# ezorita/seeq

Measured on AMD Instinct MI355X. Metric: lines/s scanned (20 bp pattern, d=3, 150 bp reads; GB/s in gb_per_s), higher is better.
Workload: dtype int (u16 automaton state ids; exact-pass columns u32 bit-vectors)

## Files before the change

### seeq_amd/csrc/seeq_pair.h

```cpp
#ifndef SEEQ_PAIR_H_
#define SEEQ_PAIR_H_

#define PAIR_X2(K) \
   asm("v_xor_b32_sdwa %0, %1, %2 dst_sel:DWORD dst_unused:UNUSED_PAD src0_sel:DWORD src1_sel:BYTE_" #K : "=v"(ada) : "v"(sa), "v"(ta)); \
   asm("v_xor_b32_sdwa %0, %1, %2 dst_sel:DWORD dst_unused:UNUSED_PAD src0_sel:DWORD src1_sel:BYTE_" #K : "=v"(adb) : "v"(sb), "v"(tb)); \
   sa = *(stream_lds_cu16 *)(uintptr_t)ada; sb = *(stream_lds_cu16 *)(uintptr_t)adb; \
   __builtin_amdgcn_sched_barrier(0);

__device__ __forceinline__ uint32_t pair_prep(uint32_t w)
{
   const uint32_t u = w & 0x06060606u;
   return u | (u << 10);
}

__device__ __forceinline__ void pair_chk(uint32_t w, uint32_t &bad, uint32_t &nm, bool first_of_two)
{
   const uint32_t idx = (w >> 1) & 0x07070707u;
   bad = __builtin_amdgcn_sad_u8(w, __builtin_amdgcn_perm(0x4EFF0AFFu, 0x47544341u, idx), bad);
   const uint32_t nf = __builtin_amdgcn_perm(0x00000100u, 0u, idx);
   nm = first_of_two ? __builtin_amdgcn_udot4(nf, 0x10204080u, nm << 8, false) : __builtin_amdgcn_udot4(nf, 0x01020408u, nm, false);
}

__device__ __forceinline__ void pair_warm4x2(uint32_t &sa, uint32_t wa, uint32_t &sb, uint32_t wb, uint32_t &seena, uint32_t &seenb)
{
   const uint32_t ta = pair_prep(wa), tb = pair_prep(wb);
   uint32_t ada, adb;
   PAIR_X2(1) asm("v_or_b32 %0, %0, %1" : "+v"(seena) : "v"(sa)); asm("v_or_b32 %0, %0, %1" : "+v"(seenb) : "v"(sb));
   PAIR_X2(3) asm("v_or_b32 %0, %0, %1" : "+v"(seena) : "v"(sa)); asm("v_or_b32 %0, %0, %1" : "+v"(seenb) : "v"(sb));
}

template <bool CHK>
__device__ __forceinline__ void pair_own4x2(uint32_t &sa, uint32_t wa, uint32_t &hma, uint32_t &nma, uint32_t &sb, uint32_t wb, uint32_t &hmb, uint32_t &nmb,
                                            uint32_t &bad, bool first_of_two)
{
   const uint32_t ta = pair_prep(wa), tb = pair_prep(wb);
   uint32_t ada, adb;
   PAIR_X2(1)
   asm volatile("" : "+v"(wa));
   if (CHK) pair_chk(wa, bad, nma, first_of_two);
   asm volatile("" : "+v"(bad), "+v"(nma));
   __builtin_amdgcn_sched_barrier(0);
   hma = __builtin_amdgcn_alignbit(sa, hma, 1); hmb = __builtin_amdgcn_alignbit(sb, hmb, 1);
   asm volatile("" : "+v"(hma), "+v"(hmb));
   PAIR_X2(3)
   asm volatile("" : "+v"(wb));
   if (CHK) pair_chk(wb, bad, nmb, first_of_two);
   asm volatile("" : "+v"(bad), "+v"(nmb));
   __builtin_amdgcn_sched_barrier(0);
   hma = __builtin_amdgcn_alignbit(sa, hma, 1); hmb = __builtin_amdgcn_alignbit(sb, hmb, 1);
   asm volatile("" : "+v"(hma), "+v"(hmb));
}

__device__ __forceinline__ uint32_t pair_word8(const fused_v4u &p, const fused_v4u &q, int k)
{
   return k == 0 ? p.x : k == 1 ? p.y : k == 2 ? p.z : k == 3 ? p.w : k == 4 ? q.x : k == 5 ? q.y : k == 6 ? q.z : q.w;
}

typedef uint32_t pair_u32_unaligned __attribute__((aligned(1)));

__device__ __forceinline__ uint32_t pair_nonbase_mask32(const fused_v4u &a, const fused_v4u &b)
{
   const uint32_t w[8] = {a.x, a.y, a.z, a.w, b.x, b.y, b.z, b.w};
   uint32_t h[2];
#pragma unroll
   for (int g = 0; g < 2; g++) {
      uint32_t acc = 0;
#pragma unroll
      for (int k = 4 * g; k < 4 * g + 4; k += 2) {
         uint32_t f[2];
#pragma unroll
         for (int u = 0; u < 2; u++) {
            const uint32_t x = w[k + u];
            const uint32_t t = x ^ __builtin_amdgcn_perm(0x474E5554u, 0x43FF41FFu, x & 0x07070707u);
            f[u] = (((t & 0x5F5F5F5Fu) + 0x7F7F7F7Fu) | t) & 0x80808080u;
         }
         acc = __builtin_amdgcn_udot4(f[0], 0x10204080u, __builtin_amdgcn_udot4(f[1], 0x01020408u, acc << 8, false), false);
      }
      h[g] = acc;
   }
   return (h[0] << 9) | (h[1] >> 7);
}

__device__ __forceinline__ uint32_t pair_count_before(const uint32_t (&m)[4], const uint32_t (&c)[5], uint32_t b)
{
   const uint32_t r = b >> 5, lz = b & 31u;
   const uint32_t mr = r == 0 ? m[0] : r == 1 ? m[1] : r == 2 ? m[2] : r == 3 ? m[3] : 0u;
   const uint32_t cr = r == 0 ? c[0] : r == 1 ? c[1] : r == 2 ? c[2] : r == 3 ? c[3] : c[4];
   return cr + (lz ? (uint32_t)__popc(mr >> (32u - lz)) : 0u);
}

template <int WU, bool CHK>
__device__ __forceinline__ void pair_walk(const fused_v4u (&v)[8], uint32_t halo, bool halo_nl, uint32_t (&hm)[2], uint32_t (&nmask)[4], uint32_t &tile_bad)
{
   constexpr int NQ = 8, NM = 4;
   uint32_t sa = 0, sb = 0, hma = 0, hmb = 0, seena = 0, seenb = 0, bad = 0, nma = 0, nmb = 0;
#pragma unroll
   for (int k = 8 - WU; k < 8; k++)
      pair_warm4x2(sa, stream_from_prev_lane(pair_word8(v[NQ - 2], v[NQ - 1], k), halo_nl ? 0x0A0A0A0Au : (uint32_t)__builtin_amdgcn_readlane((int)halo, k)),
                        sb, pair_word8(v[NQ / 2 - 2], v[NQ / 2 - 1], k), seena, seenb);
#pragma unroll
   for (int q = 0; q < NQ / 2; q++) {
      pair_own4x2<CHK>(sa, v[q].x, hma, nma, sb, v[q + NQ / 2].x, hmb, nmb, bad, true);
      pair_own4x2<CHK>(sa, v[q].y, hma, nma, sb, v[q + NQ / 2].y, hmb, nmb, bad, false);
      pair_own4x2<CHK>(sa, v[q].z, hma, nma, sb, v[q + NQ / 2].z, hmb, nmb, bad, true);
      pair_own4x2<CHK>(sa, v[q].w, hma, nma, sb, v[q + NQ / 2].w, hmb, nmb, bad, false);
      if (CHK && (q & 1)) { nmask[q >> 1] = nma; nmask[(q >> 1) + NM / 2] = nmb; nma = 0; nmb = 0; }
   }
   tile_bad = bad;
   hm[0] = __builtin_bitreverse32(hma) | ((seena & 1u) << 31);
   hm[1] = __builtin_bitreverse32(hmb) | ((seenb & 1u) << 31);
}

template <int WU, bool FA, bool IG = false, bool LL = false>
__global__ __launch_bounds__(64 * STREAM_NW, 8) void k_pair(FusedArgs a)
{
   static_assert(!(FA && IG), "SQ_IGNORE on FASTA input stays with k_stream");
   static_assert(!(LL && (FA || IG)), "the long-line variant serves plain text under SQ_FAIL / SQ_CONVERT");
   constexpr int NW = STREAM_NW;
   constexpr int CH = 128;
   constexpr int NQ = CH / 16;
   constexpr int NM = CH / 32;
   constexpr uint32_t TB = 64u * CH;
   static_assert(WU >= 4 && WU <= 8, "warm-up is 16 .. 32 bytes");
   extern __shared__ __align__(16) uint8_t dsmem[];
   const int tid = threadIdx.x, lane = tid & 63;
   const int wave = __builtin_amdgcn_readfirstlane(tid >> 6);
   {
      const fused_v4u *src = reinterpret_cast<const fused_v4u *>(a.dfa);
      for (uint32_t i = tid; i < a.dfa_rows; i += 64 * NW) reinterpret_cast<fused_v4u *>(dsmem)[i] = src[i];
   }
   __syncthreads();

   const uint32_t gwave = blockIdx.x * NW + wave, nwaves = gridDim.x * NW;
   if (a.clk_probe != nullptr && blockIdx.x == 0 && tid == 0) { a.clk_probe[0] = __builtin_readcyclecounter(); a.clk_probe[1] = wall_clock64(); }
   uint32_t wv_lines = 0, wv_hitlines = 0, wv_hdrs = 0, slice_pos = 0;
   bool wv_overflow = false;
   uint32_t wv_dirty = 0, wv_lastnl = 0;
   uint32_t dmode = 0;
   uint4 *slice = a.tmp + (size_t)gwave * a.slice_cap;
   const uint64_t lim = a.seg_base + a.seg_len;
   const uint64_t last = a.nbytes - 1;

   fused_v4u v[NQ];
   uint32_t halo = 0;
   uint32_t tile = gwave;
   while (tile < a.ntiles) {
      const uint64_t t0 = a.seg_base + (uint64_t)tile * TB;
      const bool partial = tile + 1 == a.ntiles && (a.seg_len % TB) != 0;
      const uint32_t next = tile + nwaves;
      uint32_t lane_off = (uint32_t)lane * CH;
      asm volatile("" : "+v"(lane_off));
      const uint64_t my = t0 + lane_off;
      {
         if (!partial) {
            const uint8_t *p = a.text + my;
#pragma unroll
            for (int q = 0; q < NQ; q++) v[q] = *reinterpret_cast<const fused_v4u_unaligned *>(p + 16 * q);
            uint32_t lid;
            asm volatile("v_mbcnt_lo_u32_b32 %0, -1, 0\n\tv_mbcnt_hi_u32_b32 %0, -1, %0" : "=v"(lid));
            halo = *reinterpret_cast<const pair_u32_unaligned *>(a.text + (t0 >= 32 ? t0 - 32 : 0) + ((lid & 7u) << 2));
         } else {
#pragma unroll
            for (int q = 0; q < NQ; q++) v[q] = dfa_load16(a.text, my + 16 * q, lim);
            const fused_v4u h0 = dfa_load16(a.text, t0 >= 32 ? t0 - 32 : 0, lim), h1 = dfa_load16(a.text, t0 >= 32 ? t0 - 16 : 0, lim);
            halo = pair_word8(h0, h1, 0);
#pragma unroll
            for (int k = 1; k < 8; k++) halo = (lane & 7) == k ? pair_word8(h0, h1, k) : halo;
         }
      }
      const bool halo_nl = t0 < 32;
      uint32_t hm[2], nmask[NM];
      if (!dmode) {
         uint32_t tile_bad;
         pair_walk<WU, true>(v, halo, halo_nl, hm, nmask, tile_bad);
         const uint64_t badlanes = __ballot(tile_bad != 0);
         dmode = (uint32_t)__builtin_amdgcn_readfirstlane(badlanes != 0 ? 1 : 0);
         if (LL && lane == 0) { a.tile_dirty[tile] = badlanes != 0 ? 1u : 0u; a.tile_dmask[tile] = badlanes; }
      } else {
         uint32_t unused;
         pair_walk<WU, false>(v, halo, halo_nl, hm, nmask, unused);
         if (LL && lane == 0) { a.tile_dirty[tile] = 1u; a.tile_dmask[tile] = ~0ull; }
      }
      if (dmode) {
         wv_dirty |= 1u;
#pragma unroll
         for (int r = 0; r < NM; r++) nmask[r] = stream_nl_mask32(v[2 * r], v[2 * r + 1], false);
      }
      uint32_t valid = CH;
      if (partial) {
         valid = lim > my ? (lim - my < CH ? (uint32_t)(lim - my) : (uint32_t)CH) : 0u;
#pragma unroll
         for (int r = 0; r < NM; r++) {
            const uint32_t lo = 32u * r;
            nmask[r] &= valid <= lo ? 0u : (valid >= lo + 32 ? 0xFFFFFFFFu : ~(0xFFFFFFFFu >> (valid - lo)));
         }
#pragma unroll
         for (int x = 0; x < 2; x++) {
            const uint32_t vx = valid <= 64u * x ? 0u : (valid - 64u * x >= 64u ? 64u : valid - 64u * x);
            const uint32_t np = (vx + 1u) >> 1;
            hm[x] &= np >= 32u ? 0xFFFFFFFFu : ~(0xFFFFFFFFu >> np);
         }
      }
      uint32_t mk[2] = {0u, 0u};
      const uint32_t walk_hm[2] = {hm[0], hm[1]};
      if (IG) {
         uint32_t e_tail = 0;
         if (t0 <= last && last < t0 + TB) { if (a.text[last] != '\n') e_tail = (uint32_t)(last - t0) + 1u; }
         else if (!partial && a.text[t0 + TB] == '\n') e_tail = TB;
         e_tail = (uint32_t)__builtin_amdgcn_readfirstlane((int)e_tail);
         uint32_t vm[NM], sk[NM], dn[NM];
#pragma unroll
         for (int r = 0; r < NM; r++) {
            const uint32_t lo = 32u * r;
            vm[r] = valid <= lo ? 0u : (valid >= lo + 32 ? 0xFFFFFFFFu : ~(0xFFFFFFFFu >> (valid - lo)));
            sk[r] = dmode ? pair_nonbase_mask32(v[2 * r], v[2 * r + 1]) & ~nmask[r] & vm[r] : 0u;
            dn[r] = ~(nmask[r] | sk[r]) & vm[r];
         }
         uint32_t cD[5], cS[5];
         cD[0] = 0; cS[0] = 0;
#pragma unroll
         for (int r = 0; r < NM; r++) { cD[r + 1] = cD[r] + (uint32_t)__popc(dn[r]); cS[r + 1] = cS[r] + (uint32_t)__popc(sk[r]); }
         const uint32_t end_after = (uint32_t)__builtin_amdgcn_update_dpp(0, (int)(nmask[0] >> 31), 0x130, 0xf, 0xf, true);
         uint32_t b_tail = 0;
         if (e_tail && (uint32_t)lane == (e_tail - 1u) / CH) b_tail = e_tail - (uint32_t)lane * CH;
         if (end_after) b_tail = CH;
         uint32_t baseD = 0, baseS = 0, seen_end = 0, firstP = 0, first_pq = 0;
         auto mark = [&](uint32_t pq) { if (pq < 32u) mk[0] |= 0x80000000u >> pq; else mk[1] |= 0x80000000u >> (pq - 32u); };
         auto line_end = [&](uint32_t b, uint32_t Dc, uint32_t Sc) {
            if (b >= 1u) {
               const uint32_t lineD = Dc + baseD, lineS = Sc + baseS;
               if (!seen_end) { firstP = 0x80000000u | (lineS << 14) | lineD; first_pq = (b - 1u) >> 1; }
               else if (lineS != 0u && lineD >= a.ig_thr) mark((b - 1u) >> 1);
            }
            baseD = 0u - Dc; baseS = 0u - Sc; seen_end = 1u;
         };
#pragma unroll
         for (int r = 0; r < NM; r++) {
            uint32_t mm = nmask[r];
            while (mm) {
               const uint32_t lz = (uint32_t)__builtin_clz(mm);
               mm &= ~(0x80000000u >> lz);
               line_end(32u * r + lz, cD[r] + (uint32_t)__popc((dn[r] >> 1) >> (31u - lz)), cS[r] + (uint32_t)__popc((sk[r] >> 1) >> (31u - lz)));
            }
         }
         if (__ballot(b_tail != 0u)) {
            if (b_tail == CH) line_end(CH, cD[4], cS[4]);
            else if (b_tail) line_end(b_tail, pair_count_before(dn, cD, b_tail), pair_count_before(sk, cS, b_tail));
         }
         uint32_t P = (seen_end << 31) | (cD[4] + baseD) | ((cS[4] + baseS) << 14);
#define PAIR_SEG(ctrl, rmask) { const uint32_t y = (uint32_t)__builtin_amdgcn_update_dpp(0, (int)P, ctrl, rmask, 0xf, true); P = (P >> 31) ? P : y + P; }
         PAIR_SEG(0x111, 0xf) PAIR_SEG(0x112, 0xf) PAIR_SEG(0x114, 0xf) PAIR_SEG(0x118, 0xf) PAIR_SEG(0x142, 0xa) PAIR_SEG(0x143, 0xc)
#undef PAIR_SEG
         const uint32_t starts_line = (uint32_t)__builtin_amdgcn_readfirstlane((t0 == 0 || (t0 >= 32 && ((uint32_t)__builtin_amdgcn_readlane((int)halo, 7) >> 24) == 0x0Au)) ? 1 : 0);
         const uint32_t before = stream_from_prev_lane(P, starts_line << 31);
         if ((firstP >> 31) && ((before >> 31) | starts_line)) {
            const uint32_t sum = (firstP & 0x0FFFFFFFu) + (before & 0x0FFFFFFFu);
            if ((sum >> 14) != 0u && (sum & 0x3FFFu) >= a.ig_thr) mark(first_pq);
         }
         {
            const uint32_t tile_valid = (uint32_t)__builtin_amdgcn_readfirstlane((int)(partial ? (uint32_t)(lim - t0) : TB));
            const uint32_t lv = (tile_valid - 1u) >> 7, bb = (tile_valid - 1u) & 127u;
            const uint32_t ng = (bb >> 5) == 0 ? nmask[0] : (bb >> 5) == 1 ? nmask[1] : (bb >> 5) == 2 ? nmask[2] : nmask[3];
            const uint32_t last_is_nl = (uint32_t)__builtin_amdgcn_readlane((int)((ng >> (31u - (bb & 31u))) & 1u), (int)lv);
            const bool buffer_last = t0 <= last && last < t0 + TB;
            if (!buffer_last && e_tail == 0u && !last_is_nl) {
               const uint32_t P63 = (uint32_t)__builtin_amdgcn_readlane((int)P, 63);
               const uint32_t started_here = (P63 >> 31) | starts_line;
               const uint64_t pk = t0 + tile_valid + 4u * (uint32_t)lane;
               uint32_t w = 0x0A0A0A0Au;
               if (pk + 4 <= a.nbytes) w = *reinterpret_cast<const pair_u32_unaligned *>(a.text + pk);
               else for (int i = 3; i >= 0; i--) w = (w << 8) | (pk + (uint64_t)i < a.nbytes ? (uint32_t)a.text[pk + i] : 0x0Au);
               const uint32_t nlf = nl_flags(w);
               const uint64_t nlb = __ballot(nlf != 0u);
               uint32_t qualifies = 1u;
               if (nlb != 0ull && started_here) {
                  const uint32_t F = (uint32_t)__builtin_ctzll(nlb);
                  const uint32_t nbytes_mine = (uint32_t)lane < F ? 4u : (uint32_t)lane == F ? ((uint32_t)__builtin_ctz(nlf) >> 3) : 0u;
                  const uint32_t keepm = nbytes_mine >= 4u ? 0xFFFFFFFFu : (1u << (8u * nbytes_mine)) - 1u;
                  const uint32_t y = (w ^ __builtin_amdgcn_perm(0x474E5554u, 0x43FF41FFu, w & 0x07070707u)) & keepm;
                  const uint32_t cs = (uint32_t)__popc((((y & 0x5F5F5F5Fu) + 0x7F7F7F7Fu) | y) & 0x80808080u);
                  const uint32_t tot = (uint32_t)__builtin_amdgcn_readlane((int)wave_incl_scan_u32((nbytes_mine - cs) | (cs << 16)), 63);
                  const uint32_t lineD = (P63 & 0x3FFFu) + (tot & 0xFFFFu), lineS = ((P63 >> 14) & 0x3FFFu) + (tot >> 16);
                  qualifies = (lineS != 0u && lineD >= a.ig_thr) ? 1u : 0u;
               }
               if (qualifies && (uint32_t)lane == lv) mark(bb >> 1);
            }
         }
         hm[0] |= mk[0]; hm[1] |= mk[1];
      }
      if (t0 <= last && last < t0 + TB) {
         const uint32_t o = (uint32_t)(last - t0);
         if ((uint32_t)lane == o / CH) {
            const uint32_t pos = o % CH;
#pragma unroll
            for (int r = 0; r < NM; r++)
               if ((pos >> 5) == (uint32_t)r) nmask[r] &= ~(0x80000000u >> (pos & 31));
         }
      }
      if (!LL && __ballot(((hm[0] & (hm[0] - 1u)) | (hm[1] & (hm[1] - 1u))) != 0)) {
#pragma unroll
         for (int x = 0; x < 2; x++) {
            const uint32_t n0 = nmask[2 * x], n1 = nmask[2 * x + 1], h = hm[x];
            const uint32_t f = n0 ? (uint32_t)__builtin_clz(n0) : (n1 ? 32u + (uint32_t)__builtin_clz(n1) : 64u);
            const uint32_t l = n1 ? 63u - (uint32_t)__builtin_ctz(n1) : (n0 ? 31u - (uint32_t)__builtin_ctz(n0) : 64u);
            const uint32_t na = f >= 64u ? 32u : (f + 1u) >> 1;
            const uint32_t sc = f >= 64u ? 32u : (l + 1u) >> 1;
            const uint32_t ma = na >= 32u ? 0xFFFFFFFFu : ~(0xFFFFFFFFu >> na);
            const uint32_t mc = sc >= 32u ? 0u : 0xFFFFFFFFu >> sc;
            const uint32_t ha = h & ma, hc = h & mc & ~ma;
            hm[x] = (h & ~ma & ~mc) | (ha ? (0x80000000u >> (uint32_t)__builtin_clz(ha)) | (ha & (0u - ha)) : 0u)
                                    | (hc ? (0x80000000u >> (uint32_t)__builtin_clz(hc)) | (hc & (0u - hc)) : 0u);
         }
      }
      uint32_t lane_nl = 0;
      const uint32_t lane_hits = (uint32_t)__popc(hm[0]) + (uint32_t)__popc(hm[1]);
#pragma unroll
      for (int r = 0; r < NM; r++) lane_nl += (uint32_t)__popc(nmask[r]);
      const uint32_t incl_h = wave_incl_scan_u32(lane_hits), incl_n = wave_incl_scan_u32(lane_nl);
      const uint32_t tot_h = (uint32_t)__builtin_amdgcn_readlane((int)incl_h, 63);
      const uint32_t tot_n = (uint32_t)__builtin_amdgcn_readlane((int)incl_n, 63);
      const uint32_t extra = (uint32_t)__builtin_amdgcn_readfirstlane((a.first_seg && tile == 0) ? 1 : 0);
      uint32_t dmask[NM], lane_hd = 0, excl_d = 0, tot_d = 0, hd_extra = 0;
#pragma unroll
      for (int r = 0; r < NM; r++) dmask[r] = 0;
      if (FA) {
#pragma unroll
         for (int r = 0; r < NM; r++) {
            uint32_t mm = nmask[r];
            while (mm) {
               const uint32_t lz = (uint32_t)__builtin_clz(mm);
               mm &= ~(0x80000000u >> lz);
               const uint64_t nxt = my + 32u * r + lz + 1;
               if (a.text[nxt] == '>') dmask[r] |= 0x80000000u >> lz;
            }
            lane_hd += (uint32_t)__popc(dmask[r]);
         }
         const uint32_t incl_d = wave_incl_scan_u32(lane_hd);
         excl_d = incl_d - lane_hd;
         tot_d = (uint32_t)__builtin_amdgcn_readlane((int)incl_d, 63);
         hd_extra = extra && a.text[0] == '>' ? 1u : 0u;
      }
      uint32_t incl_last = 0;
      if (tot_n && (tot_h || LL)) {
         uint32_t my_last = 0;
#pragma unroll
         for (int r = 0; r < NM; r++)
            if (nmask[r]) my_last = (uint32_t)lane * CH + 32u * r + (31u - (uint32_t)__builtin_ctz(nmask[r])) + 2u;
         incl_last = wave_incl_max_u32(my_last);
         if (LL) wv_lastnl = tile * TB + (uint32_t)__builtin_amdgcn_readlane((int)incl_last, 63) - 1u;
      }
      if (tot_h) {
         if (slice_pos + tot_h <= a.slice_cap) {
            uint32_t before = stream_from_prev_lane(incl_last, 0u);
            if (extra && before == 0) before = 1;
            if (lane_hits) {
               uint32_t ord = incl_h - lane_hits;
               uint32_t nlb = incl_n - lane_nl + extra - 1u - excl_d - hd_extra;
#pragma unroll
               for (int r = 0; r < NM; r++) {
                  uint32_t mm = (r & 1) ? hm[r >> 1] << 16 : hm[r >> 1] & 0xFFFF0000u;
                  const uint32_t mkm = (r & 1) ? mk[r >> 1] << 16 : mk[r >> 1] & 0xFFFF0000u;
                  const uint32_t wkm = (r & 1) ? walk_hm[r >> 1] << 16 : walk_hm[r >> 1] & 0xFFFF0000u;
                  while (mm) {
                     const uint32_t lp = (uint32_t)__builtin_clz(mm);
                     mm &= ~(0x80000000u >> lp);
                     const uint32_t isk = IG ? (((mkm << lp) >> 31) << 30) | ((((mkm & wkm) << lp) >> 31) << 29) : 0u;
                     uint32_t lz = 2u * lp + 1u;
                     if (partial && 32u * r + lz >= valid) lz = valid - 1u - 32u * r;
                     const uint32_t nlt = lz ? nmask[r] >> (32 - lz) : 0u;
                     const uint32_t nb = (uint32_t)__popc(nlt) - (FA && lz ? (uint32_t)__popc(dmask[r] >> (32 - lz)) : 0u);
                     const uint32_t st1 = nlt ? (uint32_t)lane * CH + 32u * r + lz - (uint32_t)__builtin_ctz(nlt) + 1u : before;
                     const uint32_t hp = (uint32_t)lane * CH + 32u * r + lz;
                     const uint32_t pos = st1 ? st1 - 1u : hp;
                     slice[slice_pos + ord] = make_uint4(tile | (st1 ? 0u : 0x80000000u) | isk, ord | ((hp - pos) << 13),
                                                         tile * TB + pos + a.pos_bias, nlb + nb);
                     ord++;
                  }
                  if (nmask[r]) before = (uint32_t)lane * CH + 32u * r + (31u - (uint32_t)__builtin_ctz(nmask[r])) + 2u;
                  nlb += (uint32_t)__popc(nmask[r]) - (uint32_t)__popc(dmask[r]);
               }
            }
            slice_pos += tot_h;
         } else {
            wv_overflow = true;
         }
      }
      if (lane == 0) {
         a.tile_cl[tile] = tot_n + extra - tot_d - hd_extra;
         a.tile_hits[tile] = tot_h;
      }
      if (!LL && tot_h && !tot_n && !partial && !(t0 <= last && last < t0 + TB)) wv_dirty |= 2u;
      wv_lines += tot_n + extra;
      wv_hdrs += tot_d + hd_extra;
      wv_hitlines += tot_h;
      tile = next;
   }
   if (lane == 0) {
      a.wg_hits[gwave] = wv_overflow ? 0u : slice_pos;
      a.wg_part[4 * gwave + 0] = wv_lines;
      a.wg_part[4 * gwave + 1] = wv_hdrs;
      if (LL) a.wg_lastnl[gwave] = wv_lastnl;
      a.wg_part[4 * gwave + 2] = wv_overflow ? (wv_hitlines | 0x80000000u) : wv_hitlines;
      a.wg_part[4 * gwave + 3] = wv_dirty;
   }   if (a.clk_probe != nullptr && blockIdx.x == 0 && tid == 0) { a.clk_probe[2] = __builtin_readcyclecounter(); a.clk_probe[3] = wall_clock64(); }
}

#undef PAIR_X2

#endif
```

Measured before the change: 26.63 billion.

## Load full tiles with coalesced 64-byte accesses and permlane transpose

Full tiles are no longer loaded as one contiguous 128-byte chunk per lane. Each group of 16 lanes now reads 64-byte pieces at strided offsets, so a wave's loads are more coalesced. permlane32/permlane16 swaps then redistribute the data so each lane still holds its own 128 bytes. A standalone microbenchmark comparing the load forms is also added. The cost is extra cross-lane swap instructions and more live registers per tile.

```diff
diff --git a/profiles/microbench/tile_layout.hip b/profiles/microbench/tile_layout.hip
--- /dev/null
+++ b/profiles/microbench/tile_layout.hip
@@ -0,0 +1,196 @@
+#include <hip/hip_runtime.h>
+#include <algorithm>
+#include <cstdio>
+#include <cstdint>
+#include <cstring>
+#include <vector>
+typedef uint32_t v4u __attribute__((ext_vector_type(4)));
+
+#define HIPCHK(x) do { hipError_t e_ = (x); if (e_ != hipSuccess) { printf("HIP error %s at line %d\n", hipGetErrorString(e_), __LINE__); return 1; } } while (0)
+
+constexpr uint32_t TILE = 8192;
+constexpr uint32_t TBL_N = 32768;
+
+__host__ __device__ inline uint32_t gen_word(uint64_t i)
+{
+   uint64_t z = (i + 1) * 0x9E3779B97F4A7C15ull; z ^= z >> 31; z *= 0xBF58476D1CE4E5B9ull; z ^= z >> 29;
+   return (uint32_t)z;
+}
+
+__global__ void k_fill(uint32_t *dst, uint64_t n)
+{
+   for (uint64_t i = (uint64_t)blockIdx.x * blockDim.x + threadIdx.x; i < n; i += (uint64_t)gridDim.x * blockDim.x) dst[i] = gen_word(i);
+}
+
+__device__ __forceinline__ void swap32(v4u &a, v4u &b)
+{
+#pragma unroll
+   for (int k = 0; k < 4; k++) { const auto r = __builtin_amdgcn_permlane32_swap(a[k], b[k], false, false); a[k] = r[0]; b[k] = r[1]; }
+}
+__device__ __forceinline__ void swap16(v4u &a, v4u &b)
+{
+#pragma unroll
+   for (int k = 0; k < 4; k++) { const auto r = __builtin_amdgcn_permlane16_swap(a[k], b[k], false, false); a[k] = r[0]; b[k] = r[1]; }
+}
+__device__ __forceinline__ void swap8(v4u &a, v4u &b, bool hi)
+{
+#pragma unroll
+   for (int k = 0; k < 4; k++) {
+      const uint32_t xa = __builtin_amdgcn_mov_dpp(a[k], 0x128, 0xf, 0xf, true), xb = __builtin_amdgcn_mov_dpp(b[k], 0x128, 0xf, 0xf, true);
+      a[k] = hi ? xb : a[k]; b[k] = hi ? b[k] : xa;
+   }
+}
+
+template <int FORM>
+__device__ __forceinline__ void load_tile(const uint8_t *t, int lane, v4u (&v)[8])
+{
+   if (FORM == 0) {
+      const uint8_t *p = t + 128u * lane;
+#pragma unroll
+      for (int q = 0; q < 8; q++) v[q] = *reinterpret_cast<const v4u *>(p + 16 * q);
+   } else if (FORM == 1) {
+      const uint8_t *p = t + 128u * (lane & 7) + 16u * (lane >> 3);
+#pragma unroll
+      for (int r = 0; r < 8; r++) v[r] = *reinterpret_cast<const v4u *>(p + 1024 * r);
+      swap32(v[0], v[4]); swap32(v[1], v[5]); swap32(v[2], v[6]); swap32(v[3], v[7]);
+      swap16(v[0], v[2]); swap16(v[1], v[3]); swap16(v[4], v[6]); swap16(v[5], v[7]);
+      const bool hi = (lane & 8) != 0;
+      swap8(v[0], v[1], hi); swap8(v[2], v[3], hi); swap8(v[4], v[5], hi); swap8(v[6], v[7], hi);
+   } else if (FORM == 2) {
+      const uint8_t *p = t + 128u * (lane & 15) + 16u * (lane >> 4);
+      v4u u[8];
+#pragma unroll
+      for (int r = 0; r < 8; r++) u[r] = *reinterpret_cast<const v4u *>(p + 2048 * (r >> 1) + 64 * (r & 1));
+      swap32(u[0], u[4]); swap32(u[1], u[5]); swap32(u[2], u[6]); swap32(u[3], u[7]);
+      swap16(u[0], u[2]); swap16(u[1], u[3]); swap16(u[4], u[6]); swap16(u[5], u[7]);
+#pragma unroll
+      for (int j = 0; j < 8; j++) v[j] = u[((j & 3) << 1) | (j >> 2)];
+   } else {
+#pragma unroll
+      for (int q = 0; q < 8; q++) v[q] = v4u{(uint32_t)(t - (const uint8_t *)0) ^ lane, 0x9E3779B9u * q + lane, (uint32_t)lane * q, 0x01010101u * q};
+   }
+}
+
+__device__ __forceinline__ void walk_word(const uint16_t *tbl, uint32_t &s, uint32_t w, uint32_t &hm, uint32_t &bad, uint32_t &nm)
+{
+   s = tbl[(s ^ w) & (TBL_N - 1)];
+   bad = __builtin_amdgcn_sad_u8(w, __builtin_amdgcn_perm(0x4EFF0AFFu, 0x47544341u, (w >> 1) & 0x07070707u), bad);
+   hm = __builtin_amdgcn_alignbit(s, hm, 1);
+   s = tbl[(s ^ (w >> 16)) & (TBL_N - 1)];
+   nm = __builtin_amdgcn_udot4(__builtin_amdgcn_perm(0x00000100u, 0u, (w >> 1) & 0x07070707u), 0x10204080u, nm << 8, false);
+   hm = __builtin_amdgcn_alignbit(s, hm, 1);
+}
+
+template <int FORM, bool CHECK>
+__global__ __launch_bounds__(1024, 8) void k_tile(const uint8_t *buf, uint32_t ntiles, uint32_t *out, unsigned long long *mismatches)
+{
+   extern __shared__ uint16_t tbl[];
+   const int tid = threadIdx.x, lane = tid & 63;
+   if (!CHECK) {
+      for (uint32_t i = tid; i < TBL_N; i += 1024) tbl[i] = (uint16_t)(gen_word(i) & (TBL_N - 1));
+      __syncthreads();
+   }
+   const uint32_t gwave = blockIdx.x * 16 + (tid >> 6), nwaves = gridDim.x * 16;
+   uint32_t acc = 0;
+   unsigned long long bad_words = 0;
+   for (uint32_t tile = gwave; tile < ntiles; tile += nwaves) {
+      const uint8_t *t = buf + (uint64_t)tile * TILE;
+      v4u v[8];
+      load_tile<FORM>(t, lane, v);
+      if (CHECK) {
+         const uint64_t w0 = ((uint64_t)tile * TILE + 128u * lane) / 4;
+#pragma unroll
+         for (int j = 0; j < 8; j++)
+#pragma unroll
+            for (int k = 0; k < 4; k++) bad_words += v[j][k] != gen_word(w0 + 4 * j + k) ? 1 : 0;
+      } else {
+         uint32_t sa = lane, sb = lane + 64, hma = 0, hmb = 0, bad = 0, nma = 0, nmb = 0;
+#pragma unroll
+         for (int q = 0; q < 4; q++)
+#pragma unroll
+            for (int k = 0; k < 4; k++) {
+               walk_word(tbl, sa, v[q][k], hma, bad, nma);
+               walk_word(tbl, sb, v[q + 4][k], hmb, bad, nmb);
+            }
+         acc += hma ^ hmb ^ bad ^ nma ^ nmb;
+      }
+   }
+   if (CHECK) { if (bad_words) atomicAdd(mismatches, bad_words); }
+   else if (lane == 0) out[gwave] = acc;
+}
+
+struct Buf { const char *name; uint8_t *p; };
+
+template <int FORM, bool CHECK>
+static void launch(const Buf &b, uint32_t ntiles, uint32_t *out, unsigned long long *mm, int grid)
+{
+   hipLaunchKernelGGL((k_tile<FORM, CHECK>), dim3(grid), dim3(1024), CHECK ? 0 : TBL_N * 2, 0, b.p, ntiles, out, mm);
+}
+
+static void launch_form(int form, bool check, const Buf &b, uint32_t ntiles, uint32_t *out, unsigned long long *mm, int grid)
+{
+   if (check) {
+      if (form == 0) launch<0, true>(b, ntiles, out, mm, grid); else if (form == 1) launch<1, true>(b, ntiles, out, mm, grid);
+      else if (form == 2) launch<2, true>(b, ntiles, out, mm, grid);
+   } else {
+      if (form == 0) launch<0, false>(b, ntiles, out, mm, grid); else if (form == 1) launch<1, false>(b, ntiles, out, mm, grid);
+      else if (form == 2) launch<2, false>(b, ntiles, out, mm, grid); else launch<3, false>(b, ntiles, out, mm, grid);
+   }
+}
+
+static const char *FORM_NAME[4] = {"(a) 128-B chunk per lane", "(b) 1 KiB coalesced + 3-stage transpose", "(c) 64-B halves + 2 permlane swaps", "walk only, no load"};
+
+int main(int argc, char **argv)
+{
+   const bool pmc = argc > 1 && !strcmp(argv[1], "pmc");
+   hipDeviceProp_t prop; HIPCHK(hipGetDeviceProperties(&prop, 0));
+   const int ncu = prop.multiProcessorCount, grid = 2 * ncu;
+   const uint64_t bytes = (uint64_t)12 << 30;
+   const uint32_t ntiles = (uint32_t)(bytes / TILE);
+   HIPCHK(hipFuncSetAttribute((const void *)k_tile<0, false>, hipFuncAttributeMaxDynamicSharedMemorySize, TBL_N * 2));
+   HIPCHK(hipFuncSetAttribute((const void *)k_tile<1, false>, hipFuncAttributeMaxDynamicSharedMemorySize, TBL_N * 2));
+   HIPCHK(hipFuncSetAttribute((const void *)k_tile<2, false>, hipFuncAttributeMaxDynamicSharedMemorySize, TBL_N * 2));
+   HIPCHK(hipFuncSetAttribute((const void *)k_tile<3, false>, hipFuncAttributeMaxDynamicSharedMemorySize, TBL_N * 2));
+   Buf bufs[2] = {{"plain 12 GiB allocation", nullptr}, {"first 12 GiB of a 16 GiB allocation", nullptr}};
+   HIPCHK(hipMalloc(&bufs[0].p, bytes));
+   HIPCHK(hipMalloc(&bufs[1].p, (size_t)16 << 30));
+   uint32_t *out; unsigned long long *mm;
+   HIPCHK(hipMalloc(&out, 4u * 16 * grid)); HIPCHK(hipMalloc(&mm, sizeof(unsigned long long)));
+   for (const Buf &b : bufs) hipLaunchKernelGGL(k_fill, dim3(4096), dim3(256), 0, 0, (uint32_t *)b.p, bytes / 4);
+   HIPCHK(hipDeviceSynchronize());
+   printf("%s, %d CUs; tiles of %u B, %u tiles per 12 GiB sweep, grid %d x 1024 threads%s\n", prop.gcnArchName, ncu, TILE, ntiles, grid, pmc ? " (pmc run: untimed)" : "");
+   int failed = 0;
+   for (const Buf &b : bufs)
+      for (int f = 0; f < 3; f++) {
+         HIPCHK(hipMemset(mm, 0, sizeof(unsigned long long)));
+         launch_form(f, true, b, ntiles, out, mm, grid);
+         unsigned long long h = 0;
+         HIPCHK(hipMemcpy(&h, mm, sizeof h, hipMemcpyDeviceToHost));
+         printf("check %-42s %-36s: %llu mismatched words of %llu\n", FORM_NAME[f], b.name, h, (unsigned long long)(bytes / 4));
+         failed |= h != 0;
+      }
+   if (failed) { printf("FAILED: a form does not give every lane bytes [128 lane, 128 lane + 128)\n"); return 2; }
+   hipEvent_t e0, e1; HIPCHK(hipEventCreate(&e0)); HIPCHK(hipEventCreate(&e1));
+   for (const Buf &b : bufs) {
+      std::vector<float> ms[4];
+      for (int f = 0; f < 4; f++) launch_form(f, false, b, ntiles, out, mm, grid);
+      HIPCHK(hipDeviceSynchronize());
+      const int rounds = pmc ? 1 : 3, reps = pmc ? 2 : 4;
+      for (int r = 0; r < rounds; r++)
+         for (int f = 0; f < 4; f++) {
+            HIPCHK(hipEventRecord(e0));
+            for (int i = 0; i < reps; i++) launch_form(f, false, b, ntiles, out, mm, grid);
+            HIPCHK(hipEventRecord(e1)); HIPCHK(hipEventSynchronize(e1));
+            float t; HIPCHK(hipEventElapsedTime(&t, e0, e1));
+            ms[f].push_back(t / reps);
+         }
+      if (pmc) continue;
+      printf("%s\n", b.name);
+      for (int f = 0; f < 4; f++) {
+         std::sort(ms[f].begin(), ms[f].end());
+         printf("  %-42s median %.3f ms per 12 GiB sweep (%.3f .. %.3f)  %.2f TB/s\n", FORM_NAME[f], ms[f][1], ms[f][0], ms[f][2], bytes / (ms[f][1] * 1e-3) / 1e12);
+      }
+   }
+   HIPCHK(hipDeviceSynchronize());
+   return 0;
+}
diff --git a/seeq_amd/csrc/seeq_pair.h b/seeq_amd/csrc/seeq_pair.h
--- a/seeq_amd/csrc/seeq_pair.h
+++ b/seeq_amd/csrc/seeq_pair.h
@@ -58,6 +58,29 @@
 
 typedef uint32_t pair_u32_unaligned __attribute__((aligned(1)));
 
+#define PAIR_TILE_LANE_OFF(l) (128u * ((l) & 15u) + 16u * ((l) >> 4))
+__device__ __forceinline__ void pair_swap32(fused_v4u &a, fused_v4u &b)
+{
+#pragma unroll
+   for (int k = 0; k < 4; k++) { const auto r = __builtin_amdgcn_permlane32_swap(a[k], b[k], false, false); a[k] = r[0]; b[k] = r[1]; }
+}
+__device__ __forceinline__ void pair_swap16(fused_v4u &a, fused_v4u &b)
+{
+#pragma unroll
+   for (int k = 0; k < 4; k++) { const auto r = __builtin_amdgcn_permlane16_swap(a[k], b[k], false, false); a[k] = r[0]; b[k] = r[1]; }
+}
+__device__ __forceinline__ void pair_load_tile(const uint8_t *t, uint32_t lane_off, fused_v4u (&v)[8])
+{
+   const uint8_t *p = t + lane_off;
+   fused_v4u u[8];
+#pragma unroll
+   for (int r = 0; r < 8; r++) u[r] = *reinterpret_cast<const fused_v4u_unaligned *>(p + 2048 * (r >> 1) + 64 * (r & 1));
+   pair_swap32(u[0], u[4]); pair_swap32(u[1], u[5]); pair_swap32(u[2], u[6]); pair_swap32(u[3], u[7]);
+   pair_swap16(u[0], u[2]); pair_swap16(u[1], u[3]); pair_swap16(u[4], u[6]); pair_swap16(u[5], u[7]);
+#pragma unroll
+   for (int j = 0; j < 8; j++) v[j] = u[((j & 3) << 1) | (j >> 2)];
+}
+
 __device__ __forceinline__ uint32_t pair_nonbase_mask32(const fused_v4u &a, const fused_v4u &b)
 {
    const uint32_t w[8] = {a.x, a.y, a.z, a.w, b.x, b.y, b.z, b.w};
@@ -153,11 +176,9 @@
       const uint64_t my = t0 + lane_off;
       {
          if (!partial) {
-            const uint8_t *p = a.text + my;
-#pragma unroll
-            for (int q = 0; q < NQ; q++) v[q] = *reinterpret_cast<const fused_v4u_unaligned *>(p + 16 * q);
             uint32_t lid;
             asm volatile("v_mbcnt_lo_u32_b32 %0, -1, 0\n\tv_mbcnt_hi_u32_b32 %0, -1, %0" : "=v"(lid));
+            pair_load_tile(a.text + t0, PAIR_TILE_LANE_OFF(lid), v);
             halo = *reinterpret_cast<const pair_u32_unaligned *>(a.text + (t0 >= 32 ? t0 - 32 : 0) + ((lid & 7u) << 2));
          } else {
 #pragma unroll
```

Result: no change. 26.44 billion (median of 6 runs) (-0.7%).
